# fthaler/cornerstone-octree

Measured on AMD Instinct MI355X. Metric: particles/sec domain.sync (encode+sort+tree+halo), 10^8 uniform, 1/2/4/8 GPU, higher is better.
Workload: dtype u64/f64

## Files before the change

cornerstone-octree_amd/csrc/ctx.hip:

```cpp
#include <dlfcn.h>

#include <algorithm>
#include <cstdio>
#include <cstdlib>
#include <cstring>
#include <mutex>
#include <unordered_set>

#include "ctx.hpp"
#include "hilbert_tables.hpp"

namespace cship
{

namespace
{
std::mutex gRegistryMutex;
std::unordered_set<const cstone_hip_ctx*>& registry()
{
    static std::unordered_set<const cstone_hip_ctx*> live;
    return live;
}

using RangePush = int (*)(const char*);
// ... 26 lines not shown
                                                   "cstone:link_octree", "cstone:halos",       "cstone:neighbors",
                                                   "cstone:minmax",      "cstone:sort_pass_iota", "cstone:resort_bins",
                                                   "cstone:resort_leaves", "cstone:gather_h",  "cstone:place",
                                                   "cstone:multipoles", "cstone:gravity", "cstone:adapt_h"};
    return stage >= 0 && stage < CSTONE_NUM_STAGES ? names[stage] : "cstone:?";
}
}

bool ctxAlive(const cstone_hip_ctx* ctx)
{
    if (!ctx) return false;
    std::lock_guard<std::mutex> lock(gRegistryMutex);
    return registry().count(ctx) != 0;
}

int ensureAuxStream(cstone_hip_ctx* ctx)
{
    if (ctx->aux) return CSTONE_OK;
    int least = 0, greatest = 0;
    CS_HIP(ctx, hipDeviceGetStreamPriorityRange(&least, &greatest));
    CS_HIP(ctx, hipStreamCreateWithPriority(&ctx->aux, hipStreamNonBlocking, least));
    CS_HIP(ctx, hipEventCreateWithFlags(&ctx->evFork, hipEventDisableTiming));
    CS_HIP(ctx, hipEventCreateWithFlags(&ctx->evJoin, hipEventDisableTiming));
    return CSTONE_OK;
}

int arenaReserve(cstone_hip_ctx* ctx, size_t totalBytes)
{
    totalBytes = alignUp(totalBytes) + 4096;
    if (totalBytes <= ctx->arenaBytes) return CSTONE_OK;
    if (ctx->arenaUsed != 0) return fail(ctx, CSTONE_E_INTERNAL, "arena grow while slices are live");
    CS_HIP(ctx, hipStreamSynchronize(ctx->stream));
    if (ctx->arena) CS_HIP(ctx, hipFree(ctx->arena));
    ctx->arena      = nullptr;
    ctx->arenaBytes = 0;
    size_t want     = totalBytes + totalBytes / 16;
    CS_HIP(ctx, hipMalloc((void**)&ctx->arena, want));
    ctx->arenaBytes = want;
    return CSTONE_OK;
}

void* arenaTake(cstone_hip_ctx* ctx, size_t bytes)
{
    size_t off = alignUp(ctx->arenaUsed);
    if (off + bytes > ctx->arenaBytes) return nullptr;
    ctx->arenaUsed = off + bytes;
// ... 119 lines not shown
int cstone_hip_ctx_destroy(cstone_hip_ctx* ctx)
{
    if (!ctx) return CSTONE_E_ARG;
    {
        std::lock_guard<std::mutex> lock(gRegistryMutex);
        if (registry().erase(ctx) == 0) return CSTONE_E_ARG;
    }
    (void)hipSetDevice(ctx->device);
    (void)hipStreamSynchronize(ctx->stream);
    for (auto& b : ctx->brackets)
    {
        (void)hipEventDestroy(b.a);
        (void)hipEventDestroy(b.b);
    }
    for (auto e : ctx->eventPool)
        (void)hipEventDestroy(e);
    if (ctx->aux)
    {
        (void)hipStreamSynchronize(ctx->aux);
        (void)hipEventDestroy(ctx->evFork);
        (void)hipEventDestroy(ctx->evJoin);
        (void)hipStreamDestroy(ctx->aux);
    }
    if (ctx->arena) (void)hipFree(ctx->arena);
    if (ctx->devScalars) (void)hipFree(ctx->devScalars);
    if (ctx->hilbertTables) (void)hipFree(ctx->hilbertTables);
    if (ctx->hostScalars) (void)hipHostFree(ctx->hostScalars);
    if (ctx->uploadStage) (void)hipHostFree(ctx->uploadStage);
    if (ctx->downloadStage) (void)hipHostFree(ctx->downloadStage);
    if (ctx->ownStream) (void)hipStreamDestroy(ctx->stream);
    delete ctx;
    return CSTONE_OK;
}

int cstone_hip_ctx_sync(cstone_hip_ctx* ctx)
{
    if (!ctx) return CSTONE_E_ARG;
    CS_TRY(copyToPinned(ctx, ctx->hostScalars + 63, ctx->devScalars + 63, sizeof(int)));
    CS_HIP(ctx, hipStreamSynchronize(ctx->stream));
    if (ctx->hostScalars[63] != 0)
    {
        (void)hipMemsetAsync(ctx->devScalars + 63, 0, sizeof(int), ctx->stream);
        return fail(ctx, CSTONE_E_INTERNAL, "device-side check failed, code 0x%x", unsigned(ctx->hostScalars[63]));
    }
    return CSTONE_OK;
}

// ... 208 lines not shown
```

cornerstone-octree_amd/csrc/ctx.hpp:

```cpp
#pragma once

#include <hip/hip_runtime.h>

#include <cstdarg>
#include <cstdio>
#include <string>
#include <vector>

#include "cstone_hip.h"

struct cstone_hip_ctx
{
    int device         = 0;
    hipStream_t stream = nullptr;
    bool ownStream     = false;
    int numCu          = 256;
    std::string lastError;

    char* arena       = nullptr;
    size_t arenaBytes = 0;
    size_t arenaUsed  = 0;

    int* hostScalars = nullptr;
    int* devScalars  = nullptr;

    char* downloadStage  = nullptr;
    char* uploadStage    = nullptr;
    size_t uploadBytes   = 0;
    size_t uploadCursor  = 0;

    hipStream_t aux    = nullptr;
    bool auxBusy       = false;
    hipEvent_t evFork  = nullptr;
    hipEvent_t evJoin  = nullptr;

    int ldsOrderOk = -1;

    void* hilbertTables = nullptr;

    int profiling  = 0;
    bool markers   = false;
    int timerDepth = 0;
    struct Bracket
    {
        int stage;
        hipEvent_t a, b;
    };
    std::vector<Bracket> brackets;
    std::vector<hipEvent_t> eventPool;
    double stageMs[CSTONE_NUM_STAGES]   = {0};
    int stageLaunches[CSTONE_NUM_STAGES] = {0};
    std::vector<float> stageSamples[CSTONE_NUM_STAGES];
};

namespace cship
{

// ... 6 lines not shown
    va_start(ap, fmt);
    vsnprintf(buf, sizeof buf, fmt, ap);
    va_end(ap);
    if (ctx) ctx->lastError = buf;
    return code;
}

#define CS_HIP(ctx, call)                                                                                              \
    do                                                                                                                 \
    {                                                                                                                  \
        hipError_t e_ = (call);                                                                                        \
        if (e_ != hipSuccess)                                                                                          \
            return cship::fail(ctx, CSTONE_E_HIP, "%s failed: %s (%s:%d)", #call, hipGetErrorString(e_), __FILE__,     \
                               __LINE__);                                                                              \
    } while (0)

#define CS_TRY(expr)                                                                                                   \
    do                                                                                                                 \
    {                                                                                                                  \
        int rc_ = (expr);                                                                                              \
        if (rc_ != CSTONE_OK) return rc_;                                                                              \
    } while (0)

int ensureAuxStream(cstone_hip_ctx* ctx);

int copyToPinned(cstone_hip_ctx* ctx, void* pinnedDst, const void* devSrc, size_t bytes);
int copyToHost(cstone_hip_ctx* ctx, void* dst, const void* devSrc, size_t bytes);
struct StreamScope
{
    cstone_hip_ctx* ctx;
    hipStream_t saved;
    StreamScope(cstone_hip_ctx* c, hipStream_t s)
        : ctx(c)
        , saved(c->stream)
    {
        ctx->stream = s;
    }
    ~StreamScope() { ctx->stream = saved; }
};

int arenaReserve(cstone_hip_ctx* ctx, size_t totalBytes);
void* arenaTake(cstone_hip_ctx* ctx, size_t bytes);
inline void arenaReset(cstone_hip_ctx* ctx) { ctx->arenaUsed = 0; }
inline size_t alignUp(size_t b, size_t a = 256) { return (b + a - 1) / a * a; }

struct StageTimer
{
    cstone_hip_ctx* ctx;
    int idx = -1;
    StageTimer(cstone_hip_ctx* c, int stage);
    ~StageTimer();
};

int minMaxCoordinates(cstone_hip_ctx* ctx, int real_bits, const void* const* xs, int numArrays, size_t n, double* out);
int minMaxCoordinatesDev(cstone_hip_ctx* ctx, int real_bits, const void* const* xs, int numArrays, size_t n,
                         double* devOut);
int extentsToReduceOperand(cstone_hip_ctx* ctx, int real_bits, const void* extents, double* devOut, double status,
                           const int* counters);

int computeKeysAndHistogram(cstone_hip_ctx* ctx, int curve, int key_bits, int real_bits, const void* x, const void* y,
                            const void* z, void* keys, size_t n, const cstone_box& box, uint32_t* hist, bool* fused,
// ... 26 lines not shown
```

cornerstone-octree_amd/csrc/domain.hip:

```cpp
#include <algorithm>
#include <cmath>
#include <cstdlib>
#include <memory>
#include <vector>

#include "ctx.hpp"
#include "devbuf.hpp"
#include "device_keys.hpp"
#include "host_tree.hpp"
#include "resort.hpp"
#include "scan.hpp"

namespace cship
{

namespace
{

template<class K>
__global__ __launch_bounds__(256) void focusOpsKernel(const K* __restrict__ prefixes,
                                                      const NodeIdx* __restrict__ childOffsets,
                                                      const NodeIdx* __restrict__ parents,
                                                      const uint32_t* __restrict__ counts, NodeIdx numNodes,
                                                      uint32_t bucket, NodeIdx* __restrict__ ops)
// ... 98 lines not shown
{
public:
    DomainImpl(cstone_hip_ctx* ctx, int curve, uint32_t bucket, uint32_t bucketFocus, float theta, const cstone_box& box)
        : ctx_(ctx)
        , curve_(curve)
        , bucket_(bucket)
        , bucketFocus_(bucketFocus)
        , theta_(theta)
        , box_(box)
    {
    }
    ~DomainImpl() override
    {
        if (pinnedLevels_) (void)hipHostFree(pinnedLevels_);
    }

    int sync(void** keysPP, void** xPP, void** yPP, void** zPP, void** hPP, size_t n, void** scratchAll, int numScratch,
             void** props, const int* propBytes, int numProps) override
    {
        if (n == 0) return fail(ctx_, CSTONE_E_ARG, "domain_sync: no particles");
        if (!firstCall_ && n != bufSize_)
            return fail(ctx_, CSTONE_E_ARG, "Domain sync: input array sizes are inconsistent (%zu != %u)", n, bufSize_);
        SyncState s{xPP, yPP, zPP, hPP, static_cast<K*>(*keysPP), n, scratchAll, numScratch, props, propBytes, numProps};
        CS_TRY(takeLevelRanges());
        CS_TRY(measureBoxFirst(s));
        CS_TRY(reserveSortBuffers(s));
        s.noOverlap   = std::getenv("CSTONE_NO_GATHER_OVERLAP") != nullptr;
        ctx_->auxBusy = false;
        CS_TRY(tryResort(s));
        resortedThisSync_ = s.sorted;
        CS_TRY(encodeSortCheckBox(s));
        CS_TRY(stepGlobalTree(s));
        CS_TRY(forkXyzGather(s, s.numAssigned));
        CS_TRY(updateFocusTree(s));
        gHost_.takeReadBack();
        CS_TRY(layoutAndHalos(s));
        CS_TRY(gatherFields(s));
        return finishSync(s);
    }

    void setHaloFactor(float factor) override { haloSearchExt_ = factor; }
    void setSortMode(int mode) override { sortMode_ = mode; }
    void setSpeculativeBox(bool on) override { speculativeBox_ = on; }
    bool maySpeculate() const { return speculativeBox_ && std::getenv("CSTONE_NO_SPECULATIVE_BOX") == nullptr; }

    int view(cstone_hip_domain_view* v) override
    {
        v->start_index           = startIndex_;
        v->end_index             = endIndex_;
        v->num_particles_with_halos = bufSize_;
        v->box                   = box_;
        v->num_global_leaves     = gLeaves_;
        v->global_leaves         = gTree_.p;
        v->global_counts         = gCounts_.as<uint32_t>();
        v->num_focus_leaves      = fLeaves_;
        v->num_focus_nodes       = fLeaves_ + (fLeaves_ - 1) / 7;
        v->focus_leaves          = fTree_.p;
        v->focus_leaf_counts     = fLeafCounts_.as<uint32_t>();
        v->prefixes              = fPrefixes_.p;
        v->child_offsets         = fChild_.as<int32_t>();
        v->parents               = fParents_.as<int32_t>();
        v->level_range           = fLevelRange_.as<int32_t>();
        v->internal_to_leaf      = fItl_.as<int32_t>();
// ... 113 lines not shown
    int sortMode_        = CSTONE_SORT_INCREMENTAL;
    bool speculativeBox_ = true;
    static constexpr int kb = 8 * sizeof(K), rb = 8 * sizeof(T);

    struct SyncState
    {
        void **xPP, **yPP, **zPP, **hPP;
        K* keys;
        size_t n;
        void** scratch;
        int numScratch;
        void** props;
        const int* propBytes;
        int numProps;
        bool speculate      = false;
        bool boxMoved       = false;
        int startPass       = 0;
        size_t sortTmpBytes = 0;
        bool sorted         = false;
        uint32_t resortMarkers = 0;
        bool fieldsMoved    = false;
        bool noOverlap      = false;
        bool xyzForked = false, xyzJoined = false;
        uint32_t numAssigned = 0;
    };

    T* extentsDev() const { return reinterpret_cast<T*>(ctx_->devScalars + 16); }
    T* extentsHost() const { return reinterpret_cast<T*>(ctx_->hostScalars + 16); }

    int takeLevelRanges()
    {
        if (!levelsPending_) return CSTONE_OK;
        CS_HIP(ctx_, hipStreamSynchronize(ctx_->stream));
        levelRangeHost_.assign(pinnedLevels_, pinnedLevels_ + maxLevel<K>() + 2);
        const int deepest = deepestLevel<K>(levelRangeHost_);
        if (deepest > deepestBound_)
            return fail(ctx_, CSTONE_E_INTERNAL, "domain_sync: the focus tree has level %d, the bound was %d", deepest,
                        deepestBound_);
        deepestBound_  = deepest;
        levelsPending_ = false;
        return CSTONE_OK;
    }

    int measureBoxFirst(SyncState& s)
    {
        const bool anyOpen = box_.bc[0] != 1 || box_.bc[1] != 1 || box_.bc[2] != 1;
// ... 39 lines not shown
    void swapFieldsWithScratch(SyncState& s, bool withH)
    {
        std::swap(*s.xPP, s.scratch[0]);
        std::swap(*s.yPP, s.scratch[1]);
        std::swap(*s.zPP, s.scratch[2]);
        if (withH) std::swap(*s.hPP, s.scratch[3]);
    }

    int forkXyzGather(SyncState& s, size_t count)
    {
        if (s.fieldsMoved || s.numScratch < 3 || s.noOverlap || s.xyzForked || count == 0) return CSTONE_OK;
        CS_TRY(ensureAuxStream(ctx_));
        CS_HIP(ctx_, hipEventRecord(ctx_->evFork, ctx_->stream));
        CS_HIP(ctx_, hipStreamWaitEvent(ctx_->aux, ctx_->evFork, 0));
        const void* src[3] = {*s.xPP, *s.yPP, *s.zPP};
        void* dst[3]       = {s.scratch[0], s.scratch[1], s.scratch[2]};
        int rc;
        {
            StreamScope scope(ctx_, ctx_->aux);
            rc = cstone_hip_gather_multi(ctx_, sizeof(T), order_.as<uint32_t>(), count, src, dst, 3);
        }
        CS_TRY(rc);
        CS_HIP(ctx_, hipEventRecord(ctx_->evJoin, ctx_->aux));
        ctx_->auxBusy = true;
        swapFieldsWithScratch(s, false);
        s.xyzForked = true;
        return CSTONE_OK;
    }
    int joinXyzGather(SyncState& s)
    {
        if (s.xyzForked && !s.xyzJoined) CS_HIP(ctx_, hipStreamWaitEvent(ctx_->stream, ctx_->evJoin, 0));
        s.xyzJoined   = true;
        ctx_->auxBusy = false;
        return CSTONE_OK;
    }

    int tryResort(SyncState& s)
    {
        const int tileLeaves = LeafResort<K>::leavesPerTile(bucketFocus_);
        const bool attempt   = !firstCall_ && tileLeaves > 0 && layoutLeaves_ == fLeaves_ && fLeaves_ > 0 &&
                             resortBackoff_ == 0 && !s.boxMoved && mayResort(sortMode_);
        if (resortBackoff_ > 0) --resortBackoff_;
        const bool fusedLeafPass = std::getenv("CSTONE_FUSED_LEAF_PASS") != nullptr;
        const bool carryFields   = s.numScratch >= 4 && fusedLeafPass;
        if (!attempt) return CSTONE_OK;
        CS_TRY(resort_.prepare(ctx_, fTree_.as<K>(), layout_.as<uint32_t>(), fLeaves_, s.n, keysAlt_.as<K>(), true,
                               carryFields ? rb : 0));
        const ResortArgs<K> ra = resort_.args();
        bool done              = false;
        CS_TRY(computeKeysResort(ctx_, curve_, kb, rb, *s.xPP, *s.yPP, *s.zPP, s.keys, s.n, box_, &ra,
                                 s.speculate ? extentsDev() : nullptr, &done));
        if (!done) return CSTONE_OK;
        CS_TRY(resort_.binMovers(ctx_, tileLeaves));
        CS_TRY(copyToPinned(ctx_, ctx_->hostScalars + 16, ctx_->devScalars + 16, 16 * sizeof(int)));
        CS_HIP(ctx_, hipStreamSynchronize(ctx_->stream));
        cstone_box next = box_;
        if (s.speculate)
        {
            double ext[6];
            for (int k = 0; k < 6; ++k)
                ext[k] = double(extentsHost()[k]);
            next = limitBoxShrinking<T>(box_, ext, firstCall_);
        }
        const bool boxChanged = !sameLimits(next, box_);
        const int* found      = ctx_->hostScalars + RESORT_SCALARS;
        const uint32_t markers = uint32_t(found[0]), J = uint32_t(found[2]), movers = uint32_t(found[3]);
        const int flags        = found[1];
        s.resortMarkers        = markers;
        if (!boxChanged && resortAccepted(flags, movers, s.n))
        {
            if (carryFields)
            {
                ResortFields rf{rb, {*s.xPP, *s.yPP, *s.zPP, *s.hPP}, {s.scratch[0], s.scratch[1], s.scratch[2], s.scratch[3]}};
                CS_TRY(resort_.sortLeavesFields(ctx_, keysAlt_.as<K>(), s.keys, order_.as<uint32_t>(), rf, movers, markers,
                                                J, tileLeaves));
                swapFieldsWithScratch(s, true);
                s.fieldsMoved = true;
            }
            else
            {
                CS_TRY(resort_.sortLeaves(ctx_, keysAlt_.as<K>(), s.keys, order_.as<uint32_t>(), movers, markers, J,
                                          tileLeaves, (flags & RESORT_LARGE_QUIET_TILES) != 0));
                CS_TRY(forkXyzGather(s, s.n - markers));
            }
            CS_HIP(ctx_, hipMemsetAsync(ctx_->devScalars + 3, 0, sizeof(int), ctx_->stream));
            s.sorted    = true;
            lastMovers_ = movers;
            ++resorts_;
            return CSTONE_OK;
        }
        if (boxChanged) { adoptChangedBox(next); }
        else
        {
            resortBackoff_ = RESORT_BACKOFF_SYNCS;
            ++resortFallbacks_;
        }
        s.speculate = false;
        return CSTONE_OK;
    }

    void adoptChangedBox(const cstone_box& next)
    {
        box_ = next;
        ++boxRedos_;
        measureFirst_ = true;
    }

    int encodeSortCheckBox(SyncState& s)
    {
        if (s.sorted) return CSTONE_OK;
        bool measured = false;
        CS_TRY(encodeAndSort(s, s.speculate, &measured));
        if (!s.speculate) return CSTONE_OK;
// ... 61 lines not shown
        return gHost_.queueReadBack(ctx_, gTree_, gCounts_, gLeaves_, true, 256);
    }

    int updateFocusTree(SyncState& s)
    {
        int conv = 0;
        if (firstCall_)
        {
            CS_TRY(ensureTree<K>(ctx_, fTree_, fLeafCounts_, fCap_, 4096));
            hipLaunchKernelGGL(initTreeKernel<K>, 1, 1, 0, ctx_->stream, fTree_.as<K>(), fLeafCounts_.as<uint32_t>(),
                               bucketFocus_ + 1);
            fLeaves_ = 1;
            CS_TRY(buildFocusOctree());
            CS_TRY(fCounts_.ensure(ctx_, sizeof(uint32_t)));
            CS_HIP(ctx_, hipMemcpyAsync(fCounts_.p, fLeafCounts_.p, sizeof(uint32_t), hipMemcpyDeviceToDevice,
                                        ctx_->stream));
            int guard = 0;
            while (!conv)
            {
                CS_TRY(updateFocus(s.keys, s.numAssigned, &conv));
                if (++guard > 64) return fail(ctx_, CSTONE_E_INTERNAL, "focus tree does not converge");
            }
        }
        return updateFocus(s.keys, s.numAssigned, &conv);
    }

    int layoutAndHalos(SyncState& s)
    {
        const NodeIdx L = fLeaves_;
        CS_TRY(layout_.ensure(ctx_, size_t(L + 1) * sizeof(uint32_t)));
        CS_TRY(radii_.ensure(ctx_, size_t(L) * sizeof(float)));
        CS_TRY(flags_.ensure(ctx_, size_t(L) * sizeof(int)));
        CS_HIP(ctx_, hipMemsetAsync(layout_.p, 0, sizeof(uint32_t), ctx_->stream));
        CS_TRY(cstone_hip_inclusive_scan_u32(ctx_, fLeafCounts_.as<uint32_t>(), layout_.as<uint32_t>() + 1, size_t(L)));
        layoutLeaves_ = L;
        static const bool splitGather = std::getenv("CSTONE_SPLIT_H_GATHER") != nullptr;
        if (s.fieldsMoved)
        {
            CS_TRY(resort_.radiiOfLeaves(ctx_, L, layout_.as<uint32_t>(), *s.hPP, rb, haloSearchExt_, radii_.as<float>()));
        }
        else
        {
            void** hDst = s.scratch;
            if (s.xyzForked && s.numScratch >= 4) { hDst = &s.scratch[3]; }
            else { CS_TRY(joinXyzGather(s)); }
            if (splitGather)
            {
// ... 36 lines not shown
        }
        for (int p = 0; p < s.numProps; ++p)
        {
            if (s.propBytes[p] > int(sizeof(T)))
                return fail(ctx_, CSTONE_E_ARG, "domain_sync: property %d is wider than the scratch element", p);
            CS_TRY(cstone_hip_gather(ctx_, s.propBytes[p], order_.as<uint32_t>(), s.numAssigned, s.props[p], *s.scratch));
            std::swap(s.props[p], *s.scratch);
        }
        return CSTONE_OK;
    }

    int finishSync(const SyncState& s)
    {
        startIndex_ = 0;
        endIndex_   = s.numAssigned;
        lastN_      = s.n;
        haveExpansion_ = false;
        bufSize_    = s.numAssigned;
        ++syncs_;
        firstCall_  = false;
#ifdef CSTONE_TEST_HOOKS
        if (std::getenv("CSTONE_FORCE_DEVICE_ERROR")) CS_HIP(ctx_, hipMemsetAsync(ctx_->devScalars + 63, 1, 1, ctx_->stream));
#endif
        return cstone_hip_ctx_sync(ctx_);
    }
    int buildFocusOctree()
    {
        const NodeIdx L = fLeaves_, M = L + (L - 1) / 7;
        CS_TRY(fPrefixes_.ensure(ctx_, size_t(M) * sizeof(K)));
        CS_TRY(fChild_.ensure(ctx_, size_t(M + 1) * sizeof(NodeIdx)));
        CS_TRY(fParents_.ensure(ctx_, size_t(std::max(1, (M - 1) / 8)) * sizeof(NodeIdx)));
        CS_TRY(fLevelRange_.ensure(ctx_, (maxLevel<K>() + 2) * sizeof(NodeIdx)));
        CS_TRY(fItl_.ensure(ctx_, size_t(M) * sizeof(NodeIdx)));
        CS_TRY(fLti_.ensure(ctx_, size_t(M) * sizeof(NodeIdx)));
        const int deepest = std::min(int(maxLevel<K>()), deepestBound_ + 1);
        CS_TRY(buildLinkedOctree(ctx_, 8 * sizeof(K), fTree_.p, L, fPrefixes_.p, fChild_.as<int32_t>(),
                                 fParents_.as<int32_t>(), fLevelRange_.as<int32_t>(), fItl_.as<int32_t>(),
                                 fLti_.as<int32_t>(), deepest));
        deepestBound_ = deepest;
        if (!pinnedLevels_)
            CS_HIP(ctx_, hipHostMalloc(reinterpret_cast<void**>(&pinnedLevels_), 32 * sizeof(NodeIdx), hipHostMallocDefault));
        CS_TRY(copyToPinned(ctx_, pinnedLevels_, fLevelRange_.p, (maxLevel<K>() + 2) * sizeof(NodeIdx)));
        levelsPending_ = true;
        return CSTONE_OK;
    }

    int updateFocus(const K* keys, size_t n, int* converged)
    {
        const NodeIdx L = fLeaves_, I = (L - 1) / 7, M = L + I;
        CS_TRY(ops_.ensure(ctx_, size_t(M + 1) * sizeof(NodeIdx)));
        CS_TRY(ops2_.ensure(ctx_, size_t(M + 1) * sizeof(NodeIdx)));
        CS_TRY(leafOps_.ensure(ctx_, size_t(L + 1) * sizeof(uint32_t)));
        int* scalars = ctx_->devScalars;
        CS_HIP(ctx_, hipMemsetAsync(scalars, 0, 2 * sizeof(int), ctx_->stream));
        hipLaunchKernelGGL(focusOpsKernel<K>, gridFor(M, 256), 256, 0, ctx_->stream, fPrefixes_.as<K>(),
                           fChild_.as<NodeIdx>(), fParents_.as<NodeIdx>(), fCounts_.as<uint32_t>(), M, bucketFocus_,
                           ops_.as<NodeIdx>());
        hipLaunchKernelGGL(protectAncestorsKernel<K>, gridFor(M, 256), 256, 0, ctx_->stream, fPrefixes_.as<K>(),
                           fParents_.as<NodeIdx>(), ops_.as<NodeIdx>(), M, ops2_.as<NodeIdx>(), scalars);
        hipLaunchKernelGGL(leafOpsKernel, gridFor(L + 1, 256), 256, 0, ctx_->stream, ops2_.as<NodeIdx>(),
                           fLti_.as<NodeIdx>(), I, L, leafOps_.as<uint32_t>());
        CS_TRY(arenaReserve(ctx_, scanArenaBytes(size_t(L) + 1)));
        int rc = scanU32(ctx_, leafOps_.as<uint32_t>(), leafOps_.as<uint32_t>(), size_t(L) + 1, 0u, false,
                         (uint32_t*)scalars + 1);
        arenaReset(ctx_);
        CS_TRY(rc);
        CS_TRY(copyToPinned(ctx_, ctx_->hostScalars, scalars, 2 * sizeof(int)));
        CS_HIP(ctx_, hipStreamSynchronize(ctx_->stream));
        *converged           = ctx_->hostScalars[0] == 0;
        const NodeIdx newL   = ctx_->hostScalars[1];
        if (newL < 1) return fail(ctx_, CSTONE_E_INTERNAL, "focus rebalance produced %d leaves", newL);

        if (!*converged)
        {
            CS_TRY(newTree_.ensure(ctx_, size_t(newL + 1) * sizeof(K)));
            CS_TRY(cstone_hip_rebalance_tree(ctx_, 8 * sizeof(K), fTree_.p, L, newL, leafOps_.as<int32_t>(),
                                             newTree_.p));
            std::swap(fTree_.p, newTree_.p);
            std::swap(fTree_.bytes, newTree_.bytes);
            CS_TRY(fLeafCounts_.ensure(ctx_, size_t(newL) * sizeof(uint32_t)));
            fCap_    = int(std::min(fTree_.bytes / sizeof(K) - 1, fLeafCounts_.bytes / sizeof(uint32_t)));
            fLeaves_ = newL;
            CS_TRY(buildFocusOctree());
        }

        const NodeIdx newI = (newL - 1) / 7, newM = newL + newI;
        const uint32_t* guess = (*converged && layoutLeaves_ == newL) ? layout_.as<uint32_t>() : nullptr;
        if (resortedThisSync_)
            CS_TRY(resort_.countLeaves(ctx_, fTree_.as<K>(), newL, keys, 0xFFFFFFFFu, fLeafCounts_.as<uint32_t>()));
        else
            CS_TRY(cstone_hip_compute_node_counts_guided(ctx_, 8 * sizeof(K), fTree_.p, fLeafCounts_.as<uint32_t>(), newL,
                                                         keys, n, 0xFFFFFFFFu, guess));
        CS_TRY(fCounts_.ensure(ctx_, size_t(newM) * sizeof(uint32_t)));
        hipLaunchKernelGGL(scatterLeafCountsKernel, gridFor(newL, 256), 256, 0, ctx_->stream,
                           fLeafCounts_.as<uint32_t>(), fLti_.as<NodeIdx>(), newI, newL, fCounts_.as<uint32_t>());
        CS_TRY(cstone_hip_upsweep_sum_bounded(ctx_, int(maxLevel<K>()) + 2, fLevelRange_.as<int32_t>(),
                                              fChild_.as<int32_t>(), fCounts_.as<uint32_t>(), deepestBound_));
        const bool sameBox = centersNodes_ == newM && sameLimits(centersBox_, box_);
        if (!(*converged && sameBox))
        {
            CS_TRY(fCenters_.ensure(ctx_, size_t(newM) * 3 * sizeof(T)));
            CS_TRY(fSizes_.ensure(ctx_, size_t(newM) * 3 * sizeof(T)));
            CS_TRY(cstone_hip_node_centers(ctx_, curve_, 8 * sizeof(K), 8 * sizeof(T), fPrefixes_.p, newM, &box_,
                                           fCenters_.p, fSizes_.p));
            centersBox_   = box_;
            centersNodes_ = newM;
        }
        CS_HIP(ctx_, hipGetLastError());
        return CSTONE_OK;
    }

    cstone_hip_ctx* ctx_;
    int curve_;
    uint32_t bucket_, bucketFocus_;
    float theta_;
    cstone_box box_;
    bool firstCall_ = true;
    uint32_t startIndex_ = 0, endIndex_ = 0, bufSize_ = 0;

    DevBuf order_, orderAlt_, keysAlt_, sortTmp_;
    LeafResort<K> resort_;
    int resortBackoff_ = 0, resorts_ = 0, resortFallbacks_ = 0;
    bool resortedThisSync_ = false;
    DevBuf gTree_, gCounts_;
    int gCap_ = 0, gLeaves_ = 0;
    GlobalTreeHost<K> gHost_;
    bool hostGlobalStep_ = std::getenv("CSTONE_DEVICE_GLOBAL_STEP") == nullptr;
    DevBuf fTree_, fLeafCounts_, fCounts_, newTree_;
    int fCap_ = 0, fLeaves_ = 0;
    int layoutLeaves_ = -1;
    cstone_box centersBox_{};
    NodeIdx centersNodes_ = -1;
    std::vector<NodeIdx> levelRangeHost_;
    NodeIdx* pinnedLevels_ = nullptr;
    bool levelsPending_    = false;
    int deepestBound_      = int(maxLevel<K>());
    int fullSortFallbacks_ = 0;
    DevBuf fPrefixes_, fChild_, fParents_, fLevelRange_, fItl_, fLti_, fCenters_, fSizes_;
    DevBuf fExpansion_;
    bool haveExpansion_ = false;
    DevBuf fMultipoles_;
    DevBuf fOctupoles_;
    DevBuf groups_;
    uint32_t numGroups_ = 0, groupsSync_ = 0;
    DevBuf ops_, ops2_, leafOps_, layout_, radii_, flags_;
};

}

using namespace cship;

struct cstone_hip_domain
{
    cstone_hip_ctx* ctx;
    std::unique_ptr<DomainBase> impl;
};

extern "C"
// ... 162 lines not shown
```

cornerstone-octree_amd/csrc/domain_mr.hip:

```cpp
#include <algorithm>
#include <chrono>
#include <cstdarg>
#include <cmath>
#include <cstdlib>
#include <limits>
#include <map>
#include <string>
#include <memory>
#include <numeric>
#include <vector>

#include "ctx.hpp"
#include "devbuf.hpp"
#include "device_keys.hpp"
#include "host_tree.hpp"
#include "let.hpp"
#include "resort.hpp"
#include "scan.hpp"

namespace cship
{

namespace
{
// ... 663 lines not shown
    std::vector<size_t> peerBytes(const uint64_t* counts, size_t stride, size_t e) const
    {
        std::vector<size_t> bytes(P_, 0);
        for (int p = 0; p < P_; ++p)
            if (p != rank_) bytes[p] = counts[p * stride] * e;
        return bytes;
    }

    int beginSync(SyncState& s, const void* mass)
    {
        if (s.massBits)
        {
            if (!useLet_) return fail(ctx_, CSTONE_E_ARG, "domain_mr_sync_grav: needs the locally essential tree (CSTONE_MR_HALOS_LET)");
            if ((s.massBits != 32 && s.massBits != 64) || s.massBits > rb || (s.n && !mass) || s.numProps < 0 || s.numProps >= MAX_PROPS)
                return fail(ctx_, CSTONE_E_ARG, "domain_mr_sync_grav: masses of 32 or 64 bits (not wider than the coordinates), "
                                                "at most %d further properties", MAX_PROPS - 1);
            for (int q = 0; q < s.numProps; ++q)
                s.propList[q] = s.props[q], s.propSizes[q] = s.propBytes[q];
            s.propList[s.numProps] = mass, s.propSizes[s.numProps] = s.massBits / 8;
            s.props = s.propList, s.propBytes = s.propSizes, ++s.numProps;
        }
        pending_ = 0, toggled_ = false;
        CS_TRY(joinPlace());
        ctx_->auxBusy = false;
        if (s.numProps < 0 || s.numProps > MAX_PROPS) setPending(CSTONE_E_ARG, "domain_mr_sync: at most %d properties", MAX_PROPS);
        for (int q = 0; q < s.numProps && !pending_; ++q)
            if ((s.n && !s.props[q]) || !gatherableElement(s.propBytes[q]))
                setPending(CSTONE_E_ARG, "domain_mr_sync: property %d must have elements of 1, 2, 4, 8, 12, 16, 24 or 32 bytes", q);
        if (s.n >= (size_t(1) << 30)) setPending(CSTONE_E_ARG, "domain_mr_sync: too many particles per rank");
        injectFailure("start");
        if (pending_)
        {
            if (P_ == 1) return agreed(rank_);
            s.n = 0, s.numProps = 0;
        }
        s.hsCounts.assign(P_, 0), s.hmatrix.assign(size_t(P_) * P_, 0);
        CS_TRY(scal_.ensure(ctx_, 4096 + size_t(P_) * (P_ + 1) * 8 + size_t(P_ + 1) * 16));
        ++syncs_;
        adapted_ = false;
        return CSTONE_OK;
    }

    int chooseBox(SyncState& s)
    {
        const bool anyOpen = !(box_.bc[0] == 1 && box_.bc[1] == 1 && box_.bc[2] == 1);
        s.resortTree = resortTree_, s.resortLeaves = resortLeaves_;
        const uint64_t layoutParticles = layoutParticles_;
// ... 259 lines not shown
                                              posB_.as<uint32_t>()));
            CS_TRY(cstone_hip_scatter(ctx_, sizeof(K), posB_.as<uint32_t>(), nb, rk_.p, s.keysM));
        }
        T* dst[4] = {o.x.as<T>() + M, o.y.as<T>() + M, o.z.as<T>() + M, o.h.as<T>() + M};
        const bool overlap = useLet_ && overlapPlace_ && !s.massBits;
        if (overlap) CS_TRY(ensureAuxStream(ctx_));
        if (overlap) placeColumns<1>(s, dst);
        else placeColumns<0>(s, dst);
        if (nb) CS_TRY(cstone_hip_scatter(ctx_, sizeof(T), posB_.as<uint32_t>(), nb, rcolS_[3].p, dst[3]));
        if (overlap)
        {
            CS_HIP(ctx_, hipEventRecord(ctx_->evFork, ctx_->stream));
            CS_HIP(ctx_, hipStreamWaitEvent(ctx_->aux, ctx_->evFork, 0));
            int rc = CSTONE_OK;
            {
                StreamScope scope(ctx_, ctx_->aux);
                placeColumns<2>(s, dst);
                for (int c = 0; c < 3 && nb && rc == CSTONE_OK; ++c)
                    rc = cstone_hip_scatter(ctx_, sizeof(T), posB_.as<uint32_t>(), nb, rcolS_[c].p, dst[c]);
            }
            CS_TRY(rc);
            CS_HIP(ctx_, hipEventRecord(ctx_->evJoin, ctx_->aux));
            placeForked_  = true;
            ctx_->auxBusy = true;
        }
        for (int c = 0; c < 3 && nb && !overlap; ++c)
            CS_TRY(cstone_hip_scatter(ctx_, sizeof(T), posB_.as<uint32_t>(), nb, rcolS_[c].p, dst[c]));
        for (int q = 0; q < s.numProps; ++q)
        {
            const int b = s.propBytes[q];
            char* to    = o.props[q].as<char>() + M * b;
            if (nb)
            {
                CS_TRY(cstone_hip_gather_scatter(ctx_, b, s.keptO, posA_.as<uint32_t>(), na, s.props[q], to));
                CS_TRY(cstone_hip_scatter(ctx_, b, posB_.as<uint32_t>(), nb, propRecvS_[q].p, to));
            }
            else { CS_TRY(cstone_hip_gather(ctx_, b, s.keptO, na, s.props[q], to)); }
        }
        return CSTONE_OK;
    }

    int ensureHostLevelRange()
    {
        if (!hostLevelRange_)
            CS_HIP(ctx_, hipHostMalloc(reinterpret_cast<void**>(&hostLevelRange_), 32 * sizeof(NodeIdx), hipHostMallocDefault));
        return CSTONE_OK;
    }
// ... 170 lines not shown
            hipLaunchKernelGGL(flaggedCountsKernel, gridFor(nLocal, 256), 256, 0, ctx_->stream, oflags_.as<int32_t>(),
                               layout_.as<uint32_t>(), first, last, cnt_.as<uint32_t>());
            CS_TRY(exclusiveScanWithTotal(cnt_.as<uint32_t>(), nLocal, scanTotal()));
            uint32_t tp = 0;
            CS_TRY(copyToHost(ctx_, &tp, scanTotal(), 4));
            if (tp)
            {
                CS_TRY(sel_.ensure(ctx_, (s.selTotal + tp) * sizeof(uint32_t), true));
                hipLaunchKernelGGL(fillIndicesKernel, gridFor(nLocal, 16), 256, 0, ctx_->stream, oflags_.as<int32_t>(),
                                   layout_.as<uint32_t>(), cnt_.as<uint32_t>(), first, last,
                                   sel_.as<uint32_t>() + s.selTotal);
            }
            s.hsCounts[p] = tp;
            s.selTotal += tp;
        }
        return CSTONE_OK;
    }

    int joinPlace()
    {
        if (!placeForked_) return CSTONE_OK;
        CS_HIP(ctx_, hipStreamWaitEvent(ctx_->stream, ctx_->evJoin, 0));
        placeForked_  = false;
        ctx_->auxBusy = false;
        return CSTONE_OK;
    }

    int shiftBlock(const SyncState& s, DevBuf& buf, size_t elem, uint64_t M2, uint64_t cap2)
    {
        const size_t bytes = s.nm * elem;
        CS_TRY(moveTmp_.ensure(ctx_, bytes));
        CS_HIP(ctx_, hipMemcpyAsync(moveTmp_.p, buf.as<char>() + s.M * elem, bytes, hipMemcpyDeviceToDevice, ctx_->stream));
        CS_TRY(buf.ensure(ctx_, cap2 * elem));
        CS_HIP(ctx_, hipMemcpyAsync(buf.as<char>() + M2 * elem, moveTmp_.p, bytes, hipMemcpyDeviceToDevice, ctx_->stream));
        return CSTONE_OK;
    }

    int makeRoomForHalos(SyncState& s)
    {
        const BlockWithHalos b = blockWithHalos(s.M, s.cap, s.nm, s.nlo, s.nhi);
        if (b.move)
        {
            Out& o = *s.o;
            CS_TRY(shiftBlock(s, o.keys, sizeof(K), b.M2, b.cap2));
            for (DevBuf* f : {&o.x, &o.y, &o.z, &o.h})
                CS_TRY(shiftBlock(s, *f, sizeof(T), b.M2, b.cap2));
            for (int q = 0; q < s.numProps; ++q)
// ... 723 lines not shown
```

cornerstone-octree_amd/csrc/sort.hip:

```cpp
#include <algorithm>
#include <cstdio>
#include <cstdlib>
#include <vector>
#include <utility>

#include "ctx.hpp"
#include "device_keys.hpp"

namespace cship
{

namespace
{

constexpr int RADIX_BITS = 8;
constexpr int RADIX      = 1 << RADIX_BITS;

constexpr uint32_t STATE_AGG  = 1u << 30;
constexpr uint32_t STATE_INC  = 2u << 30;
constexpr uint32_t COUNT_MASK = (1u << 30) - 1;

constexpr int HIST_BLOCK   = 256;
constexpr int SMALL_BLOCK  = 256;
#ifndef CSTONE_LARGE_BLOCK
// ... 928 lines not shown
    size_t need = sortTempBytes<K>(n);
    if (tempBytes < need) return fail(ctx, CSTONE_E_CAPACITY, "sort_pairs: temp %zu < %zu bytes", tempBytes, need);

    if (ctx->ldsOrderOk < 0)
    {
        uint32_t* flag = (uint32_t*)ctx->devScalars + 62;
        CS_HIP(ctx, hipMemsetAsync(flag, 0, 4, ctx->stream));
        hipLaunchKernelGGL(ldsOrderProbeKernel, 8, 1024, 0, ctx->stream, flag);
        ctx->hostScalars[62] = 1;
        CS_HIP(ctx, hipMemcpyAsync(ctx->hostScalars + 62, flag, 4, hipMemcpyDeviceToHost, ctx->stream));
        CS_HIP(ctx, hipStreamSynchronize(ctx->stream));
        ctx->ldsOrderOk = ctx->hostScalars[62] == 0;
    }
    const bool ballot = !ctx->ldsOrderOk || std::getenv("CSTONE_SORT_BALLOT_RANK") != nullptr;

    constexpr int P = sizeof(K);
    auto* words     = (uint32_t*)temp;
    SortTemp t;
    t.hist    = words;
    t.tickets = words + size_t(P) * RADIX;
    t.errors  = (uint32_t*)ctx->devScalars + 63;
    t.status  = words + headerWords(P);

    bool large       = n >= largeTileThreshold() && !ctx->auxBusy;
    size_t tile      = large ? SortCfg<K, LARGE_BLOCK>::TILE : SortCfg<K, SMALL_BLOCK>::TILE;
    size_t usedBytes = (headerWords(P) + size_t(P) * (n / tile) * RADIX) * sizeof(uint32_t);
    if (histogramState != 2) CS_HIP(ctx, hipMemsetAsync(temp, 0, usedBytes, ctx->stream));
    if (histogramState == 1) return CSTONE_OK;
    {
        StageTimer timer(ctx, CSTONE_STAGE_SORT_HIST);
        size_t nVec   = n / (16 / sizeof(K));
        unsigned grid = unsigned(std::min<size_t>(size_t(ctx->numCu) * 8, (nVec + HIST_BLOCK - 1) / HIST_BLOCK));
        grid          = std::max(grid, 1u);
        if (histogramState == 0) hipLaunchKernelGGL(histogramKernel<K>, grid, HIST_BLOCK, 0, ctx->stream, keys, n, t.hist);
        hipLaunchKernelGGL(scanHistogramKernel, P, RADIX, 0, ctx->stream, t.hist);
    }
#ifdef CSTONE_SORT_TRACE
    const char* traceFile = std::getenv("CSTONE_SORT_TRACE_FILE");
    uint64_t* traceDev    = nullptr;
    size_t traceWords     = size_t(P) * (n / tile + 1) * TRACE_SLOTS;
    if (traceFile)
    {
        CS_HIP(ctx, hipMalloc((void**)&traceDev, traceWords * 8));
        CS_HIP(ctx, hipMemsetAsync(traceDev, 0, traceWords * 8, ctx->stream));
    }
    CS_HIP(ctx, hipMemcpyToSymbolAsync(HIP_SYMBOL(g_sortTrace), &traceDev, sizeof(traceDev), 0, hipMemcpyHostToDevice,
                                       ctx->stream));
// ... 165 lines not shown
```

Measured before the change: 26.16 billion.

## Hoist focus-tree ops and rebuild onto a high-priority side stream during resort

Adds a second, high-priority 'tree' stream with its own arena, and forks the focus-tree rebalance-ops computation and tree rebuild onto it during the key encode/resort step. The host readback of the ops then overlaps the resort kernels instead of needing a separate synchronisation inside updateFocus. The hoist is skipped when the tree did not change last step. It adds error-recovery paths and a busy-mask that makes the sort fall back to the small-tile config while the side stream is active, which could cost some sort throughput.

Result: faster. 26.81 billion (median of 6 runs) (+2.5%).

```diff
diff --git a/cornerstone-octree_amd/csrc/ctx.hip b/cornerstone-octree_amd/csrc/ctx.hip
--- a/cornerstone-octree_amd/csrc/ctx.hip
+++ b/cornerstone-octree_amd/csrc/ctx.hip
@@ -72,6 +72,17 @@
     CS_HIP(ctx, hipStreamCreateWithPriority(&ctx->aux, hipStreamNonBlocking, least));
     CS_HIP(ctx, hipEventCreateWithFlags(&ctx->evFork, hipEventDisableTiming));
     CS_HIP(ctx, hipEventCreateWithFlags(&ctx->evJoin, hipEventDisableTiming));
+    return CSTONE_OK;
+}
+
+int ensureTreeStream(cstone_hip_ctx* ctx)
+{
+    if (ctx->tree) return CSTONE_OK;
+    int least = 0, greatest = 0;
+    CS_HIP(ctx, hipDeviceGetStreamPriorityRange(&least, &greatest));
+    CS_HIP(ctx, hipStreamCreateWithPriority(&ctx->tree, hipStreamNonBlocking, greatest));
+    CS_HIP(ctx, hipEventCreateWithFlags(&ctx->evTreeFork, hipEventDisableTiming));
+    CS_HIP(ctx, hipEventCreateWithFlags(&ctx->evTreeJoin, hipEventDisableTiming));
     return CSTONE_OK;
 }
 
@@ -237,7 +248,15 @@
         (void)hipEventDestroy(ctx->evJoin);
         (void)hipStreamDestroy(ctx->aux);
     }
+    if (ctx->tree)
+    {
+        (void)hipStreamSynchronize(ctx->tree);
+        (void)hipEventDestroy(ctx->evTreeFork);
+        (void)hipEventDestroy(ctx->evTreeJoin);
+        (void)hipStreamDestroy(ctx->tree);
+    }
     if (ctx->arena) (void)hipFree(ctx->arena);
+    if (ctx->sideArena) (void)hipFree(ctx->sideArena);
     if (ctx->devScalars) (void)hipFree(ctx->devScalars);
     if (ctx->hilbertTables) (void)hipFree(ctx->hilbertTables);
     if (ctx->hostScalars) (void)hipHostFree(ctx->hostScalars);
diff --git a/cornerstone-octree_amd/csrc/ctx.hpp b/cornerstone-octree_amd/csrc/ctx.hpp
--- a/cornerstone-octree_amd/csrc/ctx.hpp
+++ b/cornerstone-octree_amd/csrc/ctx.hpp
@@ -5,6 +5,7 @@
 #include <cstdarg>
 #include <cstdio>
 #include <string>
+#include <utility>
 #include <vector>
 
 #include "cstone_hip.h"
@@ -20,6 +21,9 @@
     char* arena       = nullptr;
     size_t arenaBytes = 0;
     size_t arenaUsed  = 0;
+    char* sideArena       = nullptr;
+    size_t sideArenaBytes = 0;
+    size_t sideArenaUsed  = 0;
 
     int* hostScalars = nullptr;
     int* devScalars  = nullptr;
@@ -30,9 +34,12 @@
     size_t uploadCursor  = 0;
 
     hipStream_t aux    = nullptr;
-    bool auxBusy       = false;
+    unsigned sideBusy  = 0;
     hipEvent_t evFork  = nullptr;
     hipEvent_t evJoin  = nullptr;
+    hipStream_t tree       = nullptr;
+    hipEvent_t evTreeFork  = nullptr;
+    hipEvent_t evTreeJoin  = nullptr;
 
     int ldsOrderOk = -1;
 
@@ -85,7 +92,11 @@
         if (rc_ != CSTONE_OK) return rc_;                                                                              \
     } while (0)
 
+constexpr unsigned SIDE_AUX = 1, SIDE_TREE = 2;
+constexpr int FOCUS_SCALARS = 32;
+
 int ensureAuxStream(cstone_hip_ctx* ctx);
+int ensureTreeStream(cstone_hip_ctx* ctx);
 
 int copyToPinned(cstone_hip_ctx* ctx, void* pinnedDst, const void* devSrc, size_t bytes);
 int copyToHost(cstone_hip_ctx* ctx, void* dst, const void* devSrc, size_t bytes);
@@ -93,13 +104,26 @@
 {
     cstone_hip_ctx* ctx;
     hipStream_t saved;
-    StreamScope(cstone_hip_ctx* c, hipStream_t s)
+    bool ownArena;
+    StreamScope(cstone_hip_ctx* c, hipStream_t s, bool ownArena_ = false)
         : ctx(c)
         , saved(c->stream)
+        , ownArena(ownArena_)
     {
         ctx->stream = s;
+        if (ownArena) swapArenas();
     }
-    ~StreamScope() { ctx->stream = saved; }
+    ~StreamScope()
+    {
+        if (ownArena) swapArenas();
+        ctx->stream = saved;
+    }
+    void swapArenas()
+    {
+        std::swap(ctx->arena, ctx->sideArena);
+        std::swap(ctx->arenaBytes, ctx->sideArenaBytes);
+        std::swap(ctx->arenaUsed, ctx->sideArenaUsed);
+    }
 };
 
 int arenaReserve(cstone_hip_ctx* ctx, size_t totalBytes);
diff --git a/cornerstone-octree_amd/csrc/domain.hip b/cornerstone-octree_amd/csrc/domain.hip
--- a/cornerstone-octree_amd/csrc/domain.hip
+++ b/cornerstone-octree_amd/csrc/domain.hip
@@ -144,23 +144,46 @@
         if (!firstCall_ && n != bufSize_)
             return fail(ctx_, CSTONE_E_ARG, "Domain sync: input array sizes are inconsistent (%zu != %u)", n, bufSize_);
         SyncState s{xPP, yPP, zPP, hPP, static_cast<K*>(*keysPP), n, scratchAll, numScratch, props, propBytes, numProps};
+        const int rc = runStages(s);
+        if (rc != CSTONE_OK && treeInFlight_)
+        {
+            (void)hipStreamSynchronize(ctx_->tree);
+            treeInFlight_ = false;
+        }
+        if (rc != CSTONE_OK && s.rebuilt && !s.converged && !s.treeDone)
+        {
+            firstCall_    = true;
+            layoutLeaves_ = -1;
+            deepestBound_ = int(maxLevel<K>());
+            levelRangeHost_.clear();
+        }
+        if (rc != CSTONE_OK) ctx_->sideBusy &= ~SIDE_TREE;
+        return rc;
+    }
+
+private:
+    struct SyncState;
+    int runStages(SyncState& s)
+    {
         CS_TRY(takeLevelRanges());
         CS_TRY(measureBoxFirst(s));
         CS_TRY(reserveSortBuffers(s));
-        s.noOverlap   = std::getenv("CSTONE_NO_GATHER_OVERLAP") != nullptr;
-        ctx_->auxBusy = false;
+        s.noOverlap    = std::getenv("CSTONE_NO_GATHER_OVERLAP") != nullptr;
+        s.noHoist      = std::getenv("CSTONE_NO_TREE_HOIST") != nullptr || !treeChanged_;
+        ctx_->sideBusy = 0;
         CS_TRY(tryResort(s));
         resortedThisSync_ = s.sorted;
         CS_TRY(encodeSortCheckBox(s));
         CS_TRY(stepGlobalTree(s));
         CS_TRY(forkXyzGather(s, s.numAssigned));
         CS_TRY(updateFocusTree(s));
-        gHost_.takeReadBack();
+        s.treeDone = true;
         CS_TRY(layoutAndHalos(s));
         CS_TRY(gatherFields(s));
         return finishSync(s);
     }
 
+public:
     void setHaloFactor(float factor) override { haloSearchExt_ = factor; }
     void setSortMode(int mode) override { sortMode_ = mode; }
     void setSpeculativeBox(bool on) override { speculativeBox_ = on; }
@@ -320,6 +343,14 @@
         bool fieldsMoved    = false;
         bool noOverlap      = false;
         bool xyzForked = false, xyzJoined = false;
+        bool noHoist        = false;
+        bool opsOnTree      = false;
+        bool opsTaken       = false;
+        int converged       = 0;
+        NodeIdx newL        = 0;
+        bool treeDone       = false;
+        bool hoistLate      = false;
+        bool rebuilt        = false;
         uint32_t numAssigned = 0;
     };
 
@@ -405,7 +436,7 @@
         }
         CS_TRY(rc);
         CS_HIP(ctx_, hipEventRecord(ctx_->evJoin, ctx_->aux));
-        ctx_->auxBusy = true;
+        ctx_->sideBusy |= SIDE_AUX;
         swapFieldsWithScratch(s, false);
         s.xyzForked = true;
         return CSTONE_OK;
@@ -413,8 +444,8 @@
     int joinXyzGather(SyncState& s)
     {
         if (s.xyzForked && !s.xyzJoined) CS_HIP(ctx_, hipStreamWaitEvent(ctx_->stream, ctx_->evJoin, 0));
-        s.xyzJoined   = true;
-        ctx_->auxBusy = false;
+        s.xyzJoined = true;
+        ctx_->sideBusy &= ~SIDE_AUX;
         return CSTONE_OK;
     }
 
@@ -431,12 +462,28 @@
                                carryFields ? rb : 0));
         const ResortArgs<K> ra = resort_.args();
         bool done              = false;
+        if (!s.noHoist)
+        {
+            CS_TRY(ensureTreeStream(ctx_));
+            CS_HIP(ctx_, hipEventRecord(ctx_->evTreeFork, ctx_->stream));
+        }
         CS_TRY(computeKeysResort(ctx_, curve_, kb, rb, *s.xPP, *s.yPP, *s.zPP, s.keys, s.n, box_, &ra,
                                  s.speculate ? extentsDev() : nullptr, &done));
         if (!done) return CSTONE_OK;
         CS_TRY(resort_.binMovers(ctx_, tileLeaves));
         CS_TRY(copyToPinned(ctx_, ctx_->hostScalars + 16, ctx_->devScalars + 16, 16 * sizeof(int)));
+        if (!s.noHoist)
+        {
+            s.hoistLate = std::getenv("CSTONE_TREE_HOIST_LATE") != nullptr;
+            CS_TRY(forkFocusOps(s));
+            if (!s.hoistLate)
+            {
+                CS_TRY(takeFocusOps(s));
+                CS_TRY(forkFocusRebuild(s));
+            }
+        }
         CS_HIP(ctx_, hipStreamSynchronize(ctx_->stream));
+        if (s.opsOnTree && !s.opsTaken) CS_TRY(takeFocusOps(s));
         cstone_box next = box_;
         if (s.speculate)
         {
@@ -452,6 +499,7 @@
         s.resortMarkers        = markers;
         if (!boxChanged && resortAccepted(flags, movers, s.n))
         {
+            if (s.opsTaken && markers >= s.n) return fail(ctx_, CSTONE_E_ARG, "domain_sync: all particles removed");
             if (carryFields)
             {
                 ResortFields rf{rb, {*s.xPP, *s.yPP, *s.zPP, *s.hPP}, {s.scratch[0], s.scratch[1], s.scratch[2], s.scratch[3]}};
@@ -466,12 +514,14 @@
                                           tileLeaves, (flags & RESORT_LARGE_QUIET_TILES) != 0));
                 CS_TRY(forkXyzGather(s, s.n - markers));
             }
+            if (s.opsTaken && !s.rebuilt) CS_TRY(forkFocusRebuild(s));
             CS_HIP(ctx_, hipMemsetAsync(ctx_->devScalars + 3, 0, sizeof(int), ctx_->stream));
             s.sorted    = true;
             lastMovers_ = movers;
             ++resorts_;
             return CSTONE_OK;
         }
+        if (s.rebuilt) CS_TRY(joinTreeStream());
         if (boxChanged) { adoptChangedBox(next); }
         else
         {
@@ -579,7 +629,62 @@
                 if (++guard > 64) return fail(ctx_, CSTONE_E_INTERNAL, "focus tree does not converge");
             }
         }
+        if (s.rebuilt)
+        {
+            CS_TRY(joinTreeStream());
+            return focusCounts(s.keys, s.numAssigned, s.converged);
+        }
+        if (s.opsOnTree)
+        {
+            if (!s.opsTaken) CS_TRY(takeFocusOps(s));
+            CS_TRY(focusRebuild(s.converged, s.newL));
+            return focusCounts(s.keys, s.numAssigned, s.converged);
+        }
         return updateFocus(s.keys, s.numAssigned, &conv);
+    }
+
+    int forkFocusOps(SyncState& s)
+    {
+        CS_HIP(ctx_, hipStreamWaitEvent(ctx_->tree, ctx_->evTreeFork, 0));
+        int rc;
+        {
+            StreamScope scope(ctx_, ctx_->tree, true);
+            treeInFlight_ = true;
+            rc            = focusOps();
+        }
+        CS_TRY(rc);
+        CS_HIP(ctx_, hipEventRecord(ctx_->evTreeJoin, ctx_->tree));
+        s.opsOnTree = true;
+        return CSTONE_OK;
+    }
+    int takeFocusOps(SyncState& s)
+    {
+        CS_HIP(ctx_, hipEventSynchronize(ctx_->evTreeJoin));
+        treeInFlight_ = false;
+        s.opsTaken    = true;
+        return readFocusOps(&s.converged, &s.newL);
+    }
+    int forkFocusRebuild(SyncState& s)
+    {
+        s.rebuilt = true;
+        if (s.converged) return CSTONE_OK;
+        ctx_->sideBusy |= SIDE_TREE;
+        int rc;
+        {
+            StreamScope scope(ctx_, ctx_->tree, true);
+            treeInFlight_ = true;
+            rc            = focusRebuild(s.converged, s.newL);
+        }
+        CS_TRY(rc);
+        CS_HIP(ctx_, hipEventRecord(ctx_->evTreeJoin, ctx_->tree));
+        return CSTONE_OK;
+    }
+    int joinTreeStream()
+    {
+        if (treeInFlight_) CS_HIP(ctx_, hipStreamWaitEvent(ctx_->stream, ctx_->evTreeJoin, 0));
+        treeInFlight_ = false;
+        ctx_->sideBusy &= ~SIDE_TREE;
+        return CSTONE_OK;
     }
 
     int layoutAndHalos(SyncState& s)
@@ -662,7 +767,9 @@
 #ifdef CSTONE_TEST_HOOKS
         if (std::getenv("CSTONE_FORCE_DEVICE_ERROR")) CS_HIP(ctx_, hipMemsetAsync(ctx_->devScalars + 63, 1, 1, ctx_->stream));
 #endif
-        return cstone_hip_ctx_sync(ctx_);
+        const int rc = cstone_hip_ctx_sync(ctx_);
+        if (rc != CSTONE_E_HIP) gHost_.takeReadBack();
+        return rc;
     }
     int buildFocusOctree()
     {
@@ -687,11 +794,21 @@
 
     int updateFocus(const K* keys, size_t n, int* converged)
     {
+        CS_TRY(focusOps());
+        CS_HIP(ctx_, hipStreamSynchronize(ctx_->stream));
+        NodeIdx newL = 0;
+        CS_TRY(readFocusOps(converged, &newL));
+        CS_TRY(focusRebuild(*converged, newL));
+        return focusCounts(keys, n, *converged);
+    }
+
+    int focusOps()
+    {
         const NodeIdx L = fLeaves_, I = (L - 1) / 7, M = L + I;
         CS_TRY(ops_.ensure(ctx_, size_t(M + 1) * sizeof(NodeIdx)));
         CS_TRY(ops2_.ensure(ctx_, size_t(M + 1) * sizeof(NodeIdx)));
         CS_TRY(leafOps_.ensure(ctx_, size_t(L + 1) * sizeof(uint32_t)));
-        int* scalars = ctx_->devScalars;
+        int* scalars = ctx_->devScalars + FOCUS_SCALARS;
         CS_HIP(ctx_, hipMemsetAsync(scalars, 0, 2 * sizeof(int), ctx_->stream));
         hipLaunchKernelGGL(focusOpsKernel<K>, gridFor(M, 256), 256, 0, ctx_->stream, fPrefixes_.as<K>(),
                            fChild_.as<NodeIdx>(), fParents_.as<NodeIdx>(), fCounts_.as<uint32_t>(), M, bucketFocus_,
@@ -705,27 +822,36 @@
                          (uint32_t*)scalars + 1);
         arenaReset(ctx_);
         CS_TRY(rc);
-        CS_TRY(copyToPinned(ctx_, ctx_->hostScalars, scalars, 2 * sizeof(int)));
-        CS_HIP(ctx_, hipStreamSynchronize(ctx_->stream));
-        *converged           = ctx_->hostScalars[0] == 0;
-        const NodeIdx newL   = ctx_->hostScalars[1];
-        if (newL < 1) return fail(ctx_, CSTONE_E_INTERNAL, "focus rebalance produced %d leaves", newL);
-
-        if (!*converged)
-        {
-            CS_TRY(newTree_.ensure(ctx_, size_t(newL + 1) * sizeof(K)));
-            CS_TRY(cstone_hip_rebalance_tree(ctx_, 8 * sizeof(K), fTree_.p, L, newL, leafOps_.as<int32_t>(),
-                                             newTree_.p));
-            std::swap(fTree_.p, newTree_.p);
-            std::swap(fTree_.bytes, newTree_.bytes);
-            CS_TRY(fLeafCounts_.ensure(ctx_, size_t(newL) * sizeof(uint32_t)));
-            fCap_    = int(std::min(fTree_.bytes / sizeof(K) - 1, fLeafCounts_.bytes / sizeof(uint32_t)));
-            fLeaves_ = newL;
-            CS_TRY(buildFocusOctree());
-        }
-
-        const NodeIdx newI = (newL - 1) / 7, newM = newL + newI;
-        const uint32_t* guess = (*converged && layoutLeaves_ == newL) ? layout_.as<uint32_t>() : nullptr;
+        return copyToPinned(ctx_, ctx_->hostScalars + FOCUS_SCALARS, scalars, 2 * sizeof(int));
+    }
+
+    int readFocusOps(int* converged, NodeIdx* newL)
+    {
+        *converged = ctx_->hostScalars[FOCUS_SCALARS] == 0;
+        *newL      = ctx_->hostScalars[FOCUS_SCALARS + 1];
+        if (*newL < 1) return fail(ctx_, CSTONE_E_INTERNAL, "focus rebalance produced %d leaves", *newL);
+        return CSTONE_OK;
+    }
+
+    int focusRebuild(int converged, NodeIdx newL)
+    {
+        if (converged) return CSTONE_OK;
+        const NodeIdx L = fLeaves_;
+        CS_TRY(newTree_.ensure(ctx_, size_t(newL + 1) * sizeof(K)));
+        CS_TRY(cstone_hip_rebalance_tree(ctx_, 8 * sizeof(K), fTree_.p, L, newL, leafOps_.as<int32_t>(), newTree_.p));
+        std::swap(fTree_.p, newTree_.p);
+        std::swap(fTree_.bytes, newTree_.bytes);
+        CS_TRY(fLeafCounts_.ensure(ctx_, size_t(newL) * sizeof(uint32_t)));
+        fCap_    = int(std::min(fTree_.bytes / sizeof(K) - 1, fLeafCounts_.bytes / sizeof(uint32_t)));
+        fLeaves_ = newL;
+        return buildFocusOctree();
+    }
+
+    int focusCounts(const K* keys, size_t n, int converged)
+    {
+        const NodeIdx newL = fLeaves_, newI = (newL - 1) / 7, newM = newL + newI;
+        treeChanged_       = !converged;
+        const uint32_t* guess = (converged && layoutLeaves_ == newL) ? layout_.as<uint32_t>() : nullptr;
         if (resortedThisSync_)
             CS_TRY(resort_.countLeaves(ctx_, fTree_.as<K>(), newL, keys, 0xFFFFFFFFu, fLeafCounts_.as<uint32_t>()));
         else
@@ -737,7 +863,7 @@
         CS_TRY(cstone_hip_upsweep_sum_bounded(ctx_, int(maxLevel<K>()) + 2, fLevelRange_.as<int32_t>(),
                                               fChild_.as<int32_t>(), fCounts_.as<uint32_t>(), deepestBound_));
         const bool sameBox = centersNodes_ == newM && sameLimits(centersBox_, box_);
-        if (!(*converged && sameBox))
+        if (!(converged && sameBox))
         {
             CS_TRY(fCenters_.ensure(ctx_, size_t(newM) * 3 * sizeof(T)));
             CS_TRY(fSizes_.ensure(ctx_, size_t(newM) * 3 * sizeof(T)));
@@ -774,6 +900,8 @@
     std::vector<NodeIdx> levelRangeHost_;
     NodeIdx* pinnedLevels_ = nullptr;
     bool levelsPending_    = false;
+    bool treeChanged_      = true;
+    bool treeInFlight_     = false;
     int deepestBound_      = int(maxLevel<K>());
     int fullSortFallbacks_ = 0;
     DevBuf fPrefixes_, fChild_, fParents_, fLevelRange_, fItl_, fLti_, fCenters_, fSizes_;
diff --git a/cornerstone-octree_amd/csrc/domain_mr.hip b/cornerstone-octree_amd/csrc/domain_mr.hip
--- a/cornerstone-octree_amd/csrc/domain_mr.hip
+++ b/cornerstone-octree_amd/csrc/domain_mr.hip
@@ -709,7 +709,7 @@
         }
         pending_ = 0, toggled_ = false;
         CS_TRY(joinPlace());
-        ctx_->auxBusy = false;
+        ctx_->sideBusy &= ~SIDE_AUX;
         if (s.numProps < 0 || s.numProps > MAX_PROPS) setPending(CSTONE_E_ARG, "domain_mr_sync: at most %d properties", MAX_PROPS);
         for (int q = 0; q < s.numProps && !pending_; ++q)
             if ((s.n && !s.props[q]) || !gatherableElement(s.propBytes[q]))
@@ -1015,7 +1015,7 @@
             CS_TRY(rc);
             CS_HIP(ctx_, hipEventRecord(ctx_->evJoin, ctx_->aux));
             placeForked_  = true;
-            ctx_->auxBusy = true;
+            ctx_->sideBusy |= SIDE_AUX;
         }
         for (int c = 0; c < 3 && nb && !overlap; ++c)
             CS_TRY(cstone_hip_scatter(ctx_, sizeof(T), posB_.as<uint32_t>(), nb, rcolS_[c].p, dst[c]));
@@ -1232,7 +1232,7 @@
         if (!placeForked_) return CSTONE_OK;
         CS_HIP(ctx_, hipStreamWaitEvent(ctx_->stream, ctx_->evJoin, 0));
         placeForked_  = false;
-        ctx_->auxBusy = false;
+        ctx_->sideBusy &= ~SIDE_AUX;
         return CSTONE_OK;
     }
 
diff --git a/cornerstone-octree_amd/csrc/sort.hip b/cornerstone-octree_amd/csrc/sort.hip
--- a/cornerstone-octree_amd/csrc/sort.hip
+++ b/cornerstone-octree_amd/csrc/sort.hip
@@ -974,7 +974,7 @@
     t.errors  = (uint32_t*)ctx->devScalars + 63;
     t.status  = words + headerWords(P);
 
-    bool large       = n >= largeTileThreshold() && !ctx->auxBusy;
+    bool large       = n >= largeTileThreshold() && ctx->sideBusy == 0;
     size_t tile      = large ? SortCfg<K, LARGE_BLOCK>::TILE : SortCfg<K, SMALL_BLOCK>::TILE;
     size_t usedBytes = (headerWords(P) + size_t(P) * (n / tile) * RADIX) * sizeof(uint32_t);
     if (histogramState != 2) CS_HIP(ctx, hipMemsetAsync(temp, 0, usedBytes, ctx->stream));
```
